# tictacmenthe/F2CNN

Measured on AMD Instinct MI355X. Metric: audio-seconds/sec through filterbank+envelope (HIP, 1 MI355X per rank); the +CNN figure of BASELINE's metric is value_with_cnn / blocks.cfg4, higher is better.
Workload: dtype f64 filter state + f64 utterance FFT + f32 row FFT; 1 GPU; cfg3: filterbank + Hilbert envelope + 50 Hz LPF in one call (f32 FFT), batch of 1000 x 1 s utterances per GPU, 128 channels, ENV1 (float64) out; channels=128, lpf_hz=50, launch_batch=1000, outputs_resident_in_hbm=True, parallelism=utterance-sharded x1, no collective, utterances_sent_back_by_the_accuracy_guard=0

## Files before the change

### f2cnn_amd/csrc/f2_fft13_merged.h

```cpp
#pragma once
template <int NT, int PTV>
__device__ __forceinline__ void fft13_pass12_merged(cpx<float>* lds, const cpx<float>* twl, int tid, cpx<float> (&v)[PTV]) {
    constexpr int LOG2H = 13;
    static_assert(NT == 512 && PTV >= 16 && plan_npass(LOG2H) == 4 && plan_bits(LOG2H, 1) == 3 && plan_bits(LOG2H, 2) == 2 &&
                      plan_bits(LOG2H, 0) == 4, "the 16-8-4-16 plan on 512 threads");
    constexpr int OFF2 = plan_tw_offset(LOG2H, 2) - plan_tw_offset(LOG2H, 1);
    const int l = tid & 63, hl = l >> 5;
    const int base8 = (l & 31) + 32 * (tid >> 6);
#pragma unroll
    for (int i = 0; i < 2; ++i) {
        const int b = base8 + 256 * (i + 2 * hl);
        const cpx<float>* src = lds + cpad(b);
#pragma unroll
        for (int j = 0; j < 8; ++j) v[i * 8 + j] = src[j * (1024 + 64)];
    }
    __syncthreads();
#pragma unroll
    for (int i = 0; i < 2; ++i) {
        dft<8>(&v[i * 8]);
        const cpx<float>* t1 = twl + (((base8 >> 4) + 16 * (i + 2 * hl)));
#pragma unroll
        for (int k = 1; k < 8; ++k) v[i * 8 + brev<8>(k)] = cmul(v[i * 8 + brev<8>(k)], t1[(k - 1) * 64]);
    }
#pragma unroll
    for (int i = 0; i < 2; ++i) {
        cpx<float>& A0 = v[i * 8 + brev<8>(0)];
        cpx<float>& B0 = v[i * 8 + brev<8>(4)];
        cpx<float>& A1 = v[i * 8 + brev<8>(1)];
        cpx<float>& B1 = v[i * 8 + brev<8>(5)];
        cpx<float>& A2 = v[i * 8 + brev<8>(2)];
        cpx<float>& B2 = v[i * 8 + brev<8>(6)];
        cpx<float>& A3 = v[i * 8 + brev<8>(3)];
        cpx<float>& B3 = v[i * 8 + brev<8>(7)];
        asm volatile("s_nop 1\n\t"
                     "v_permlane32_swap_b32 %0, %1\n\t"
                     "v_permlane32_swap_b32 %2, %3\n\t"
                     "v_permlane32_swap_b32 %4, %5\n\t"
                     "v_permlane32_swap_b32 %6, %7\n\t"
                     "v_permlane32_swap_b32 %8, %9\n\t"
                     "v_permlane32_swap_b32 %10, %11\n\t"
                     "v_permlane32_swap_b32 %12, %13\n\t"
                     "v_permlane32_swap_b32 %14, %15\n\t"
                     "s_nop 1"
                     : "+v"(A0.re), "+v"(B0.re), "+v"(A0.im), "+v"(B0.im), "+v"(A1.re), "+v"(B1.re), "+v"(A1.im), "+v"(B1.im),
                       "+v"(A2.re), "+v"(B2.re), "+v"(A2.im), "+v"(B2.im), "+v"(A3.re), "+v"(B3.re), "+v"(A3.im), "+v"(B3.im));
    }
    const int q = base8 & 15, plo = base8 >> 4;
    const cpx<float>* t2 = twl + OFF2 + plo;
#pragma unroll
    for (int k = 0; k < 4; ++k) {
        cpx<float> t[4] = {v[brev<8>(k)], v[8 + brev<8>(k)], v[brev<8>(k + 4)], v[8 + brev<8>(k + 4)]};
        dft<4>(t);
        const int pos = q + 16 * (k + 4 * hl) + 512 * plo;
        lds[cpad(pos)] = t[0];
#pragma unroll
        for (int k2 = 1; k2 < 4; ++k2) lds[cpad(pos + 128 * k2)] = cmul(t[brev<4>(k2)], t2[(k2 - 1) * 16]);
    }
    __syncthreads();
}

#define F2_SWAP8(OP, a0, b0, a1, b1, a2, b2, a3, b3, a4, b4, a5, b5, a6, b6, a7, b7)                                        \
    asm volatile("s_nop 1\n\t" OP " %0, %1\n\t" OP " %2, %3\n\t" OP " %4, %5\n\t" OP " %6, %7\n\t" OP " %8, %9\n\t" OP      \
                 " %10, %11\n\t" OP " %12, %13\n\t" OP " %14, %15\n\ts_nop 1"                                                \
                 : "+v"(a0), "+v"(b0), "+v"(a1), "+v"(b1), "+v"(a2), "+v"(b2), "+v"(a3), "+v"(b3), "+v"(a4), "+v"(b4),       \
                   "+v"(a5), "+v"(b5), "+v"(a6), "+v"(b6), "+v"(a7), "+v"(b7))
template <int NT, int PTV>
__device__ __forceinline__ void fft14_pass12_merged(cpx<float>* lds, const cpx<float>* twl, int tid, cpx<float> (&v)[PTV]) {
    constexpr int LOG2H = 14;
    static_assert(NT == 1024 && PTV >= 16 && plan_npass(LOG2H) == 4 && plan_bits(LOG2H, 0) == 4 && plan_bits(LOG2H, 1) == 4 &&
                      plan_bits(LOG2H, 2) == 2 && plan_bits(LOG2H, 3) == 4, "the 16-16-4-16 plan on 1024 threads");
    constexpr int OFF2 = plan_tw_offset(LOG2H, 2) - plan_tw_offset(LOG2H, 1);
    const int l = tid & 63, wv = tid >> 6;
    const int x = l & 15, jp = l >> 4;
    const int b = x + 16 * (wv + 16 * jp);
    const cpx<float>* src = lds + cpad(b);
#pragma unroll
    for (int j = 0; j < 16; ++j) v[j] = src[j * (1024 + 64)];
    __syncthreads();
    dft<16>(&v[0]);
    const cpx<float>* t1 = twl + (wv + 16 * jp);
#pragma unroll
    for (int k = 1; k < 16; ++k) v[brev<16>(k)] = cmul(v[brev<16>(k)], t1[(k - 1) * 64]);
#define F2_S(k) v[brev<16>(k)]
    F2_SWAP8("v_permlane32_swap_b32", F2_S(0).re, F2_S(8).re, F2_S(0).im, F2_S(8).im, F2_S(1).re, F2_S(9).re, F2_S(1).im, F2_S(9).im,
             F2_S(2).re, F2_S(10).re, F2_S(2).im, F2_S(10).im, F2_S(3).re, F2_S(11).re, F2_S(3).im, F2_S(11).im);
    F2_SWAP8("v_permlane32_swap_b32", F2_S(4).re, F2_S(12).re, F2_S(4).im, F2_S(12).im, F2_S(5).re, F2_S(13).re, F2_S(5).im,
             F2_S(13).im, F2_S(6).re, F2_S(14).re, F2_S(6).im, F2_S(14).im, F2_S(7).re, F2_S(15).re, F2_S(7).im, F2_S(15).im);
    F2_SWAP8("v_permlane16_swap_b32", F2_S(0).re, F2_S(4).re, F2_S(0).im, F2_S(4).im, F2_S(1).re, F2_S(5).re, F2_S(1).im, F2_S(5).im,
             F2_S(2).re, F2_S(6).re, F2_S(2).im, F2_S(6).im, F2_S(3).re, F2_S(7).re, F2_S(3).im, F2_S(7).im);
    F2_SWAP8("v_permlane16_swap_b32", F2_S(8).re, F2_S(12).re, F2_S(8).im, F2_S(12).im, F2_S(9).re, F2_S(13).re, F2_S(9).im,
             F2_S(13).im, F2_S(10).re, F2_S(14).re, F2_S(10).im, F2_S(14).im, F2_S(11).re, F2_S(15).re, F2_S(11).im, F2_S(15).im);
    const int kk0 = 4 * (jp & 1) + 8 * (jp >> 1);
    const cpx<float>* t2 = twl + OFF2 + wv;
#pragma unroll
    for (int k = 0; k < 4; ++k) {
        cpx<float> t[4] = {F2_S(k), F2_S(k + 4), F2_S(k + 8), F2_S(k + 12)};
        dft<4>(t);
        const int pos = x + 16 * (k + kk0) + 1024 * wv;
        lds[cpad(pos)] = t[0];
#pragma unroll
        for (int k2 = 1; k2 < 4; ++k2) lds[cpad(pos + 256 * k2)] = cmul(t[brev<4>(k2)], t2[(k2 - 1) * 16]);
    }
#undef F2_S
    __syncthreads();
}

template <int LOG2H, int NT, int PTV>
__device__ __forceinline__ void fft_pass0_pair(const cpx<float>* __restrict__ tw, int tid, cpx<float> (&va)[PTV], cpx<float> (&vb)[PTV]) {
    constexpr int R = 16, NB = (1 << LOG2H) / R;
    static_assert(NT == NB && PTV == R && plan_bits(LOG2H, 0) == 4, "one radix-16 butterfly per thread");
    dft<R>(&va[0]);
    dft<R>(&vb[0]);
    const cpx<float>* twq = tw + plan_tw_offset(LOG2H, 0) + tid;
    cpx<float> w[R];
    w[1] = twq[0];
    w[4] = twq[3 * NB];
    w[2] = cmul(w[1], w[1]);
    w[3] = cmul(w[2], w[1]);
    w[8] = cmul(w[4], w[4]);
    w[5] = cmul(w[4], w[1]);
    w[6] = cmul(w[4], w[2]);
    w[7] = cmul(w[4], w[3]);
    w[12] = cmul(w[8], w[4]);
    w[9] = cmul(w[8], w[1]);
    w[10] = cmul(w[8], w[2]);
    w[11] = cmul(w[8], w[3]);
    w[13] = cmul(w[12], w[1]);
    w[14] = cmul(w[12], w[2]);
    w[15] = cmul(w[12], w[3]);
#pragma unroll
    for (int k = 1; k < R; ++k) {
        va[brev<R>(k)] = cmul(va[brev<R>(k)], w[k]);
        vb[brev<R>(k)] = cmul(vb[brev<R>(k)], w[k]);
    }
}

template <int LOG2H, int PTV, int NT, bool T0REGS, int PASS = 1>
__device__ __forceinline__ void fft_remaining_passes(cpx<float>* lds, const cpx<float>* __restrict__ tw, const cpx<float>* twl, int tid,
                                                     cpx<float> (&v)[PTV]) {
    constexpr int NP = plan_npass(LOG2H);
    if constexpr (PASS < NP) {
        fft_pass<float, LOG2H, PASS, false, PASS == NP - 1, PTV, NT, false, T0REGS>(lds, tw, twl, tid, v);
        fft_remaining_passes<LOG2H, PTV, NT, T0REGS, PASS + 1>(lds, tw, twl, tid, v);
    }
}
template <int LOG2H, int PTV, int NT, bool T0REGS>
__device__ __forceinline__ void fft_from_pass0(cpx<float>* lds, const cpx<float>* __restrict__ tw, const cpx<float>* twl, int tid,
                                               cpx<float> (&v)[PTV]) {
#pragma unroll
    for (int k = 0; k < 16; ++k) lds[cpad(tid * 16 + k)] = v[brev<16>(k)];
    __syncthreads();
    if constexpr (LOG2H == 13) {
        fft13_pass12_merged<NT, PTV>(lds, twl, tid, v);
        fft_pass<float, 13, 3, false, true, PTV, NT, false, T0REGS>(lds, tw, twl, tid, v);
    } else if constexpr (LOG2H == 14) {
        fft14_pass12_merged<NT, PTV>(lds, twl, tid, v);
        fft_pass<float, 14, 3, false, true, PTV, NT, false, T0REGS>(lds, tw, twl, tid, v);
    } else {
        fft_remaining_passes<LOG2H, PTV, NT, T0REGS>(lds, tw, twl, tid, v);
    }
}

template <int PTV, int NT, bool T0REGS>
__device__ __forceinline__ void fft13_regs_to_regs(cpx<float>* lds, const cpx<float>* __restrict__ tw, const cpx<float>* twl, int tid,
                                                   cpx<float> (&v)[PTV]) {
    fft_pass<float, 13, 0, true, false, PTV, NT, false, T0REGS>(lds, tw, twl, tid, v);
    fft13_pass12_merged<NT, PTV>(lds, twl, tid, v);
    fft_pass<float, 13, 3, false, true, PTV, NT, false, T0REGS>(lds, tw, twl, tid, v);
}
```

### f2cnn_amd/csrc/f2_fft_lds.h

```cpp
#pragma once
#include <cmath>
#include <vector>

#include "f2_envelope_core.h"

namespace f2fft {

constexpr int THREADS13 = 512;
constexpr int MINWAVES13 = 4;
template <typename F>
constexpr int threads_for(int log2h) {
    return (log2h == 14 && sizeof(F) == 4) ? 1024 : (log2h == 13 && sizeof(F) == 4) ? THREADS13 : log2h >= 13 ? 512 : 256;
}
template <typename F, int LOG2H>
constexpr int threads_for() { return threads_for<F>(LOG2H); }
template <typename F, int LOG2H>
constexpr int min_waves_for() {
    return (sizeof(F) == 4 && LOG2H == 13) ? MINWAVES13 : (sizeof(F) == 4 && LOG2H == 14) ? 4 : 2;
}

template <typename F, int LOG2H>
constexpr bool derive_tw0() { return sizeof(F) == 4 && LOG2H >= 11 && LOG2H <= 14; }

constexpr int FUSE_HILBERT_MAX = 12;
template <typename F, int LOG2H>
constexpr bool fuse_hilbert() { return LOG2H >= 1 && LOG2H <= FUSE_HILBERT_MAX && sizeof(F) == 4; }

constexpr int plan_npass(int h, int p13 = 4) {
    return h == 0 ? 0 : h <= 5 ? 1 : h <= 10 ? ((h & 1) ? 3 : 2) : (h == 13 && p13 == 4) ? 4 : h == 14 ? 4 : 3;
}
constexpr int plan_bits(int h, int pass, int p13 = 4) {
    if (h <= 5) return h;
    if (h <= 10) return (h & 1) ? (pass == 1 ? 1 : (h - 1) / 2) : h / 2;
    if (h == 13 && p13 == 4) return pass == 1 ? 3 : pass == 2 ? 2 : 4;
    if (h == 14) return pass == 2 ? 2 : 4;
    const int a = h <= 13 ? 4 : 5;
    return pass == 1 ? h - 2 * a : a;
}
constexpr int plan_points_per_thread(int h, int nt, int p13 = 4) {
    int m = 1;
    for (int p = 0; p < plan_npass(h, p13); ++p) {
        const int R = 1 << plan_bits(h, p, p13);
        const int nb = (1 << h) / R;
        const int pts = ((nb + nt - 1) / nt) * R;
        m = pts > m ? pts : m;
    }
    return m;
}
constexpr int plan_shift(int h, int pass, int p13 = 4) {
    int s = 0;
    for (int i = 0; i < pass; ++i) s += plan_bits(h, i, p13);
    return s;
}
constexpr int plan_tw_count(int h, int pass, int p13 = 4) {
    const int R = 1 << plan_bits(h, pass, p13), S = 1 << plan_shift(h, pass, p13), H = 1 << h;
    return S * R == H ? 0 : (R - 1) * (H / R / S);
}
constexpr int plan_tw_offset(int h, int pass, int p13 = 4) {
    int o = 0;
    for (int i = 0; i < pass; ++i) o += plan_tw_count(h, i, p13);
    return o;
}
constexpr int plan_tw_total(int h, int p13 = 4) { return plan_tw_offset(h, plan_npass(h, p13), p13); }
constexpr int plan_tw_lds_count(int h, int p13 = 4) { return plan_npass(h, p13) >= 2 ? plan_tw_total(h, p13) - plan_tw_offset(h, 1, p13) : 0; }

__device__ __forceinline__ int cpad(int i) { return i + (i >> 4); }
constexpr int cpad_size(int h) { return h + (h >> 4) + 1; }

template <typename F, int LOG2H, int PASS, bool SRC_REGS, bool DST_REGS, int PTV, int NT, bool HILBERT = false,
          bool T0REGS = false, int P13 = 4>
__device__ __forceinline__ void fft_pass(cpx<F>* lds, const cpx<F>* __restrict__ tw, const cpx<F>* twl, int tid,
                                         cpx<F> (&v)[PTV]) {
    constexpr int H = 1 << LOG2H;
    constexpr int R = 1 << plan_bits(LOG2H, PASS, P13);
    constexpr int LOG2S = plan_shift(LOG2H, PASS, P13);
    constexpr int S = 1 << LOG2S;
    constexpr int NB = H / R;
    constexpr int ITER = (NB + NT - 1) / NT;
    constexpr bool LAST = (S * R == H);
    static_assert(ITER * R <= PTV, "register array too small");
    constexpr bool FULL = NB % NT == 0;
    const cpx<F>* __restrict__ twp = tw + plan_tw_offset(LOG2H, PASS, P13);
    if constexpr (!SRC_REGS) {
#pragma unroll
        for (int i = 0; i < ITER; ++i) {
            const int bf = tid + i * NT;
            if (FULL || bf < NB) {
                if constexpr (NB % 16 == 0) {
                    const cpx<F>* src = lds + cpad(bf);
#pragma unroll
                    for (int j = 0; j < R; ++j) v[i * R + j] = src[j * (NB + NB / 16)];
                } else {
#pragma unroll
                    for (int j = 0; j < R; ++j) v[i * R + j] = lds[cpad(bf + j * NB)];
                }
                if constexpr (HILBERT) {
                    const cpx<F>* __restrict__ V = tw + plan_tw_total(LOG2H, P13);
                    const F sc = F(1.0 / H);
#pragma unroll
                    for (int j = 0; j < R; ++j) {
                        const int m = bf + j * NB;
                        const cpx<F> zp = (NB % 16 == 0) ? (lds + cpad(H - bf))[-j * (NB + NB / 16)] : lds[cpad(H - m)];
                        const bool upper = 2 * m > H;
                        const cpx<F> vk = V[upper ? H - m : m];
                        const F cs = (upper ? -vk.re : vk.re) * sc, sn = -vk.im * sc;
                        const cpx<F> z = v[i * R + j];
                        const F wre = cs * zp.re - sn * z.im, wim = sn * z.re - cs * zp.im;
                        v[i * R + j] = {m == 0 ? F(0) : wre, m == 0 ? F(0) : -wim};
                    }
                }
            }
        }
        __syncthreads();
    }
#pragma unroll
    for (int i = 0; i < ITER; ++i) {
        const int bf = tid + i * NT;
        if (FULL || bf < NB) {
            dft<R>(&v[i * R]);
            if constexpr (!LAST) {
                const cpx<F>* twq = (PASS >= 1 ? twl + (plan_tw_offset(LOG2H, PASS, P13) - plan_tw_offset(LOG2H, 1, P13)) : twp) +
                                    (bf >> LOG2S);
                if constexpr (PASS == 0 && T0REGS && R == 16) {
                    cpx<F> w[R];
                    w[1] = twq[0];
                    w[4] = twq[3 * (NB / S)];
                    w[2] = cmul(w[1], w[1]);
                    w[3] = cmul(w[2], w[1]);
                    w[8] = cmul(w[4], w[4]);
                    w[5] = cmul(w[4], w[1]);
                    w[6] = cmul(w[4], w[2]);
                    w[7] = cmul(w[4], w[3]);
                    w[12] = cmul(w[8], w[4]);
                    w[9] = cmul(w[8], w[1]);
                    w[10] = cmul(w[8], w[2]);
                    w[11] = cmul(w[8], w[3]);
                    w[13] = cmul(w[12], w[1]);
                    w[14] = cmul(w[12], w[2]);
                    w[15] = cmul(w[12], w[3]);
#pragma unroll
                    for (int k = 1; k < R; ++k) v[i * R + brev<R>(k)] = cmul(v[i * R + brev<R>(k)], w[k]);
                } else {
#pragma unroll
                    for (int k = 1; k < R; ++k)
                        v[i * R + brev<R>(k)] = cmul(v[i * R + brev<R>(k)], twq[(k - 1) * (NB / S)]);
                }
            }
            if constexpr (!DST_REGS) {
                const int q = bf & (S - 1);
                const int base = q + (bf - q) * R;
                if constexpr (S % 16 == 0) {
                    cpx<F>* dst = lds + cpad(base);
#pragma unroll
                    for (int k = 0; k < R; ++k) dst[k * (S + S / 16)] = v[i * R + brev<R>(k)];
                } else {
#pragma unroll
                    for (int k = 0; k < R; ++k) lds[cpad(base + S * k)] = v[i * R + brev<R>(k)];
                }
            }
        }
    }
    if constexpr (!DST_REGS) __syncthreads();
}

template <typename F, int LOG2H, bool INVERSE, int PTV, int NT, bool T0REGS = false, int PASS = 0, int P13 = 4>
__device__ __forceinline__ void fft_all(cpx<F>* lds, const cpx<F>* __restrict__ tw, const cpx<F>* twl, int tid,
                                        cpx<F> (&v)[PTV]) {
    constexpr int NP = plan_npass(LOG2H, P13);
    if constexpr (PASS < NP) {
        constexpr bool SRC = !INVERSE && PASS == 0;
        constexpr bool DST = INVERSE && PASS == NP - 1;
// ... 46 lines not shown
```

### f2cnn_amd/csrc/f2_spectral.hip

```cpp
#include <algorithm>
#include <cmath>
#include <complex>
#include <thread>

#include "f2_fft_lds.h"

using namespace f2fft;

namespace {

typedef float f2_f4 __attribute__((ext_vector_type(4)));
constexpr int SPEC_GB = 16;

constexpr int KS_CGROUP = 32;
constexpr int KS_CGROUP_LONG = 8;
constexpr int KS_STORE_AUX = 2;
typedef unsigned int f2_u4 __attribute__((ext_vector_type(4)));
typedef unsigned int f2_u2 __attribute__((ext_vector_type(2)));
__device__ __forceinline__ __amdgpu_buffer_rsrc_t row_buffer(double* y, int n) {
    return __builtin_amdgcn_make_buffer_rsrc(y, 0, n * 8, 0x00020000);
}
__device__ __forceinline__ __amdgpu_buffer_rsrc_t row_buffer_uniform(double* y, int n) {
    const unsigned long long a = (unsigned long long)y;
    const unsigned lo = __builtin_amdgcn_readfirstlane((unsigned)a), hi = __builtin_amdgcn_readfirstlane((unsigned)(a >> 32));
    return row_buffer((double*)(((unsigned long long)hi << 32) | lo), __builtin_amdgcn_readfirstlane(n));
}
__device__ __forceinline__ void store_row_pair_inside(__amdgpu_buffer_rsrc_t r, int i0, double a, double b) {
    const f2_d2 v = {a, b};
    __builtin_amdgcn_raw_buffer_store_b128(__builtin_bit_cast(f2_u4, v), r, i0 * 8, 0, KS_STORE_AUX);
}
__device__ __forceinline__ void store_row_pair_buf(__amdgpu_buffer_rsrc_t r, int n, int i0, double a, double b) {
    if (i0 + 1 < n) {
        const f2_d2 v = {a, b};
        __builtin_amdgcn_raw_buffer_store_b128(__builtin_bit_cast(f2_u4, v), r, i0 * 8, 0, KS_STORE_AUX);
    } else if (i0 < n) {
        __builtin_amdgcn_raw_buffer_store_b64(__builtin_bit_cast(f2_u2, a), r, i0 * 8, 0, KS_STORE_AUX);
    }
}
__device__ __forceinline__ void store_row_pair_front(__amdgpu_buffer_rsrc_t r, int t0, double a, double b) {
    if (t0 >= 0) {
        const f2_d2 v = {a, b};
        __builtin_amdgcn_raw_buffer_store_b128(__builtin_bit_cast(f2_u4, v), r, t0 * 8, 0, KS_STORE_AUX);
    } else if (t0 == -1) {
        __builtin_amdgcn_raw_buffer_store_b64(__builtin_bit_cast(f2_u2, b), r, 0, 0, KS_STORE_AUX);
    }
}

struct LowpassConsts {
    float qf, b0f;
    float g1, g2, g4, g8;
    double gw, gblk;
};

template <int NT, int NBLK>
constexpr size_t lowpass_tab_lds_bytes() {
    return sizeof(float) * (2 * (size_t)NBLK * (NT / 64) + NBLK);
}

#define F2_DPP_STEP(CTRL)                                                                                                    \
    asm volatile("s_nop 1\n\t"                                                                                               \
                 "v_fmac_f32_dpp %0, %0, %16 " CTRL "\n\t"                                                                   \
                 "v_fmac_f32_dpp %1, %1, %16 " CTRL "\n\t"                                                                   \
                 "v_fmac_f32_dpp %2, %2, %16 " CTRL "\n\t"                                                                   \
                 "v_fmac_f32_dpp %3, %3, %16 " CTRL "\n\t"                                                                   \
                 "v_fmac_f32_dpp %4, %4, %16 " CTRL "\n\t"                                                                   \
                 "v_fmac_f32_dpp %5, %5, %16 " CTRL "\n\t"                                                                   \
                 "v_fmac_f32_dpp %6, %6, %16 " CTRL "\n\t"                                                                   \
                 "v_fmac_f32_dpp %7, %7, %16 " CTRL "\n\t"                                                                   \
                 "v_fmac_f32_dpp %8, %8, %16 " CTRL "\n\t"                                                                   \
                 "v_fmac_f32_dpp %9, %9, %16 " CTRL "\n\t"                                                                   \
                 "v_fmac_f32_dpp %10, %10, %16 " CTRL "\n\t"                                                                 \
                 "v_fmac_f32_dpp %11, %11, %16 " CTRL "\n\t"                                                                 \
                 "v_fmac_f32_dpp %12, %12, %16 " CTRL "\n\t"                                                                 \
                 "v_fmac_f32_dpp %13, %13, %16 " CTRL "\n\t"                                                                 \
                 "v_fmac_f32_dpp %14, %14, %16 " CTRL "\n\t"                                                                 \
                 "v_fmac_f32_dpp %15, %15, %16 " CTRL                                                                        \
                 : "+v"(sc[0]), "+v"(sc[1]), "+v"(sc[2]), "+v"(sc[3]), "+v"(sc[4]), "+v"(sc[5]), "+v"(sc[6]), "+v"(sc[7]),   \
                   "+v"(sc[8]), "+v"(sc[9]), "+v"(sc[10]), "+v"(sc[11]), "+v"(sc[12]), "+v"(sc[13]), "+v"(sc[14]), "+v"(sc[15]) \
                 : "v"(mult))

template <int NT, int NBLK, bool CHAINED = false, bool INSIDE_BUT_FIRST = false>
__device__ __forceinline__ float lowpass_pairs_store_tab(const float (&er)[NBLK], const float (&ei)[NBLK], const LowpassConsts& K,
                                                        const f2_f4* __restrict__ lptab, unsigned char* smem,
                                                        double* __restrict__ y, int n, int tid, int ibase = 0,
                                                        double* ychain = nullptr, int np = 0) {
    static_assert(NBLK == 16, "sixteen blocks: one DPP row chains them");
// ... 176 lines not shown
    asm volatile("s_nop 1\n\t"                                         \
                 "v_max_f32_dpp %0, %0, %0 " CTRL "\n\t"               \
                 "v_max_f32_dpp %1, %1, %1 " CTRL                       \
                 : "+v"(a), "+v"(b))
__device__ __forceinline__ void wave_max63x2(float& a, float& b) {
    F2_DPP_MAX2("row_shr:1 row_mask:0xf bank_mask:0xf bound_ctrl:0");
    F2_DPP_MAX2("row_shr:2 row_mask:0xf bank_mask:0xf bound_ctrl:0");
    F2_DPP_MAX2("row_shr:4 row_mask:0xf bank_mask:0xf bound_ctrl:0");
    F2_DPP_MAX2("row_shr:8 row_mask:0xf bank_mask:0xf bound_ctrl:0");
    F2_DPP_MAX2("row_bcast:15 row_mask:0xa bank_mask:0xf");
    F2_DPP_MAX2("row_bcast:31 row_mask:0xc bank_mask:0xf");
}
__device__ __forceinline__ float wave_max63(float v) {
    asm volatile("s_nop 1\n\t"
                 "v_max_f32_dpp %0, %0, %0 row_shr:1 row_mask:0xf bank_mask:0xf bound_ctrl:0\n\ts_nop 1\n\t"
                 "v_max_f32_dpp %0, %0, %0 row_shr:2 row_mask:0xf bank_mask:0xf bound_ctrl:0\n\ts_nop 1\n\t"
                 "v_max_f32_dpp %0, %0, %0 row_shr:4 row_mask:0xf bank_mask:0xf bound_ctrl:0\n\ts_nop 1\n\t"
                 "v_max_f32_dpp %0, %0, %0 row_shr:8 row_mask:0xf bank_mask:0xf bound_ctrl:0\n\ts_nop 1\n\t"
                 "v_max_f32_dpp %0, %0, %0 row_bcast:15 row_mask:0xa bank_mask:0xf\n\ts_nop 1\n\t"
                 "v_max_f32_dpp %0, %0, %0 row_bcast:31 row_mask:0xc bank_mask:0xf"
                 : "+v"(v));
    return v;
}

template <int R0, int NT, bool PADFIRST>
__device__ __forceinline__ float pad_residual(const cpx<float> (&v)[R0], int np, int tid, int odd, float gout) {
    if constexpr (PADFIRST) {
        return fmaxf(gout, 2 * tid + odd < np ? fabsf(v[brev<R0>(0)].re) : 0.f);
    } else {
        int jlim = (np - 2 * tid - odd + 2 * NT - 1) >> (__builtin_ctz(2 * NT));
        asm volatile("" : "+v"(jlim));
#pragma unroll
        for (int j = 0; j < R0 / 2; ++j) gout = fmaxf(gout, j < jlim ? fabsf(v[brev<R0>(j)].re) : 0.f);
        return gout;
    }
}

template <int NT, int NBLK, bool FIRSTONLY>
__device__ __forceinline__ void zero_front_padding(float (&er)[NBLK], float (&ei)[NBLK], int np, int tid) {
    int d = 2 * tid - np;
    asm volatile("" : "+v"(d));
#pragma unroll
    for (int jj = 0; jj < (FIRSTONLY ? 1 : NBLK / 2); ++jj) {
        er[jj] = d >= -2 * NT * jj ? er[jj] : 0.f;
        ei[jj] = d >= -2 * NT * jj - 1 ? ei[jj] : 0.f;
    }
}

#ifdef F2_STAMPS
#define F2_STAMP_STORE_ROW(st, N, out, row)                                                             \
    do {                                                                                                \
        if (threadIdx.x == 0 && (out))                                                                  \
            for (int k_ = 0; k_ < (N); ++k_) (out)[(size_t)(row) * (N) + k_] = (st)[k_];                \
    } while (0)
#else
#define F2_STAMP_STORE_ROW(st, N, out, row) \
    do {                                    \
    } while (0)
#endif

__device__ __forceinline__ void guard_decide(const SpecParams& P, const unsigned* guard, int b, int c) {
    const float gi = __uint_as_float(guard[0]), go = __uint_as_float(guard[1]), gl = __uint_as_float(guard[2]);
    const float den = P.lpf ? gl : gi;
    const bool flag = go > P.tol * den;
    if (flag) P.uflag[b] = 1;
    if (P.gdump) {
        float* g = P.gdump + ((size_t)b * (size_t)P.C + (size_t)c) * 4;
        g[0] = gi;
        g[1] = go;
        g[2] = gl;
        g[3] = flag ? 1.f : 0.f;
    }
}

template <int LOG2H, bool PADFIRST>
__global__ __launch_bounds__((threads_for<float, LOG2H>()), (min_waves_for<float, LOG2H>())) void k_spectral_envelope(
    const cpx<float>* __restrict__ Xall , const f2_f4* __restrict__ HUall,
    const cpx<float>* __restrict__ E , const float* __restrict__ rho_all ,
    const int64_t* __restrict__ offsets, const int* __restrict__ ulist, const cpx<float>* __restrict__ tw,
    const f2_f4* __restrict__ lptab, SpecParams P) {
    constexpr int NT = threads_for<float, LOG2H>();
    constexpr int H = 1 << LOG2H;
    constexpr int M = 2 * H;
    constexpr int CS = cpad_size(H);
    constexpr int R0 = 1 << plan_bits(LOG2H, 0);
    constexpr int NB0 = H / R0;
    static_assert(NB0 % NT == 0, "every thread owns whole butterflies of the first pass");
    constexpr int ITER0 = NB0 / NT;
    constexpr int PT = plan_points_per_thread(LOG2H, NT);
    constexpr int NBLK = ITER0 * R0;
    static_assert(PT == NBLK, "register shape");
    constexpr size_t LP = lowpass_tab_lds_bytes<NT, NBLK>();
    constexpr int LDS_BYTES = (int)((size_t)CS * 8 > LP ? (size_t)CS * 8 : LP);
    __shared__ __attribute__((aligned(16))) unsigned char smem[LDS_BYTES];
    constexpr int TWL = plan_tw_lds_count(LOG2H);
    __shared__ __attribute__((aligned(16))) cpx<float> twl[TWL > 0 ? TWL : 1];
    __shared__ unsigned guard[4];
    cpx<float>* lds = reinterpret_cast<cpx<float>*>(smem);

    const int tid = threadIdx.x;
    int u, c;
    row_decode<KS_CGROUP>(P, u, c);
    const int row_id = u * P.C + c;
    const float* __restrict__ rho_g = rho_all + (size_t)row_id * 8;
    const cpx<float>* __restrict__ Xu = Xall + (size_t)((unsigned long long)(unsigned)u * P.xpitch);
    const f2_f4* __restrict__ HUc = HUall + (size_t)((unsigned long long)(unsigned)c * P.tpitch);

    F2_STAMP_ARRAY(st, 8);
    F2_STAMP(st, 0);
    if (tid < 4) guard[tid] = 0u;

    static_assert(ITER0 == 1 && R0 == 16, "one radix-16 butterfly per thread in the first pass");
    constexpr int GB = SPEC_GB, NG = R0 / GB;
    cpx<float> yk[PT], v[PT];
    static_assert(NB0 == NT && plan_npass(LOG2H) >= 3, "fft_pass0_pair + fft_from_pass0");
    cpx<float> vo[PT];
    cpx<float> w0 = E[tid];
    constexpr int TWIT = (TWL + NT - 1) / NT;
    cpx<float> twr[TWIT > 0 ? TWIT : 1];
    {
        unsigned tw1 = plan_tw_offset(LOG2H, 1) * (unsigned)sizeof(cpx<float>);
        asm volatile("" : "+s"(tw1));
#pragma unroll
        for (int it = 0; it < TWIT; ++it) {
            const unsigned i = (it + 1) * NT <= TWL ? (unsigned)(tid + it * NT) : min((unsigned)(tid + it * NT), (unsigned)(TWL - 1));
            twr[it] = *reinterpret_cast<const cpx<float>*>(reinterpret_cast<const char*>(tw) + (i * (unsigned)sizeof(cpx<float>) + tw1));
        }
    }
    const cpx<float> XH = Xu[H];
    const f2_f4 HUH = HUc[H];
    float rho[8];
#pragma unroll
    for (int q = 0; q < 8; ++q) rho[q] = rho_g[q];
    cpx<float> Xl[2][GB];
    f2_f4 Hl[2][GB];
    unsigned kb8 = (unsigned)tid * (unsigned)sizeof(cpx<float>);
    asm volatile("" : "+v"(kb8));
    const __amdgpu_buffer_rsrc_t Xb = table_buffer(Xu, (H + 1) * (int)sizeof(cpx<float>)), HUb = table_buffer(HUc, (H + 1) * (int)sizeof(f2_f4));
    int b = 0;
#pragma unroll
    for (int qq = 0; qq < GB; ++qq) {
        const int q = qq == 0 ? 0 : qq == 1 ? GB - 1 : qq - 1;
        Xl[0][q] = lane_load<cpx<float>>(Xb, kb8, q * NB0);
        Hl[0][q] = lane_load<f2_f4>(HUb, 2 * kb8, q * NB0);
        __builtin_amdgcn_sched_barrier(0);
        if (qq == 0) {
            int u_late = u;
            asm volatile("" : "+s"(u_late));
            b = ulist[u_late];
        }
    }
    float nyq[6] = {XH.re, XH.im, HUH.x, HUH.y, HUH.z, HUH.w};
    asm volatile("" : "+s"(nyq[0]), "+s"(nyq[1]), "+s"(nyq[2]), "+s"(nyq[3]), "+s"(nyq[4]), "+s"(nyq[5]));
    asm volatile("" : "+s"(rho[0]), "+s"(rho[1]), "+s"(rho[2]), "+s"(rho[3]), "+s"(rho[4]), "+s"(rho[5]), "+s"(rho[6]), "+s"(rho[7]));
#pragma unroll
    for (int it = 0; it < TWIT; ++it) twl[(it + 1) * NT <= TWL ? tid + it * NT : min(tid + it * NT, TWL - 1)] = twr[it];
    asm volatile("" : "+s"(b));
    const int64_t off = offsets[b];
    const int n = (int)(offsets[b + 1] - off);
    const int np = M - n;
    double* __restrict__ y = P.env + ((size_t)P.C * (size_t)off + (size_t)c * (size_t)n);
#pragma unroll
    for (int g = 0; g < NG; ++g) {
        if (g + 1 < NG) {
#pragma unroll
            for (int q = 0; q < GB; ++q) {
                Xl[(g + 1) & 1][q] = lane_load<cpx<float>>(Xb, kb8, ((g + 1) * GB + q) * NB0);
                Hl[(g + 1) & 1][q] = lane_load<f2_f4>(HUb, 2 * kb8, ((g + 1) * GB + q) * NB0);
            }
        }
#pragma unroll
        for (int q = 0; q < GB; ++q) {
            const int j = g * GB + q;
            const cpx<float> wj = bin_w<R0>(w0, j);
            yk[j] = spectral_bin(Xl[g & 1][q], Hl[g & 1][q], wj, rho);
            vo[j] = {yk[j].re * wj.re + yk[j].im * wj.im, yk[j].re * wj.im - yk[j].im * wj.re};
#ifdef F2_STAMPS
            if (j == 0 || j == 7) {
                asm volatile("s_nop 0" : "+v"(yk[j].re), "+v"(yk[j].im));
                st[j == 0 ? 1 : 2] = __builtin_amdgcn_s_memrealtime();
                asm volatile("s_nop 0" : "+v"(yk[j].re));
            }
#endif
        }
        asm volatile("" : "+v"(kb8), "+v"(w0.re), "+v"(w0.im), "+v"(yk[g * GB].re), "+v"(yk[g * GB + GB - 1].re));
    }
#ifdef F2_STAMPS
    asm volatile("s_nop 0" : "+v"(yk[15].re), "+v"(yk[15].im));
    st[3] = __builtin_amdgcn_s_memrealtime();
    asm volatile("s_nop 0" : "+v"(yk[15].re));
#endif
    if (tid == 0) {
        const cpx<float> yh = spectral_bin(cpx<float>{nyq[0], nyq[1]}, f2_f4{nyq[2], nyq[3], nyq[4], nyq[5]}, cpx<float>{-1.f, 0.f}, rho);
        yk[0] = {yk[0].re, yh.re};
    }
    float er[NBLK], ei[NBLK];
    float gin = 0.f, gout = 0.f;
    constexpr bool T0R = derive_tw0<float, LOG2H>();
    {
#pragma unroll
        for (int j = 0; j < R0; ++j) v[j] = {yk[j].re, -yk[j].im};
        if (tid == 0) {
            v[0] = {0.5f * (yk[0].re + yk[0].im), 0.f};
            vo[0] = {0.5f * (yk[0].re - yk[0].im), 0.f};
        }
        F2_STAMP(st, 4);
        int tid_e = tid;
        asm volatile("" : "+v"(tid_e), "+v"(v[0].re), "+v"(vo[PT - 1].im));
        fft_pass0_pair<LOG2H, NT, PT>(tw, tid_e, v, vo);
        fft_from_pass0<LOG2H, PT, NT, T0R>(lds, tw, twl, tid_e, v);
        gout = pad_residual<R0, NT, PADFIRST>(v, np, tid, 0, gout);
#pragma unroll
        for (int j = 0; j < R0; ++j) {
            const cpx<float> a = v[brev<R0>(j)];
            er[j] = fsqrt(a.re * a.re + a.im * a.im);
        }
        fft_from_pass0<LOG2H, PT, NT, T0R>(lds, tw, twl, tid_e, vo);
        F2_STAMP(st, 5);
        gout = pad_residual<R0, NT, PADFIRST>(vo, np, tid, 1, gout);
#pragma unroll
        for (int j = 0; j < R0; ++j) {
            const cpx<float> a = vo[brev<R0>(j)];
            ei[j] = fsqrt(a.re * a.re + a.im * a.im);
        }
    }
    zero_front_padding<NT, NBLK, PADFIRST>(er, ei, np, tid);
#pragma unroll
    for (int jj = 0; jj < NBLK; ++jj) gin = fmaxf(gin, fmaxf(er[jj], ei[jj]));
    float glp = 0.f;
    wave_max63x2(gin, gout);
    if ((tid & 63) == 63) {
        __hip_atomic_fetch_max(&guard[0], __float_as_uint(gin), __ATOMIC_RELAXED, __HIP_MEMORY_SCOPE_WORKGROUP);
        __hip_atomic_fetch_max(&guard[1], __float_as_uint(gout), __ATOMIC_RELAXED, __HIP_MEMORY_SCOPE_WORKGROUP);
    }
    F2_STAMP(st, 6);
    if (!P.lpf) {
        const __amdgpu_buffer_rsrc_t yb = row_buffer(y, n);
#pragma unroll
        for (int jj = 0; jj < NBLK; ++jj) {
            const int t0 = 2 * (tid + NT * jj) - np;
            if ((PADFIRST && jj > 0) || jj >= NBLK / 2 || 2 * NT * jj >= np) store_row_pair_inside(yb, t0, (double)er[jj], (double)ei[jj]);
            else if (2 * NT * (jj + 1) > np) store_row_pair_front(yb, t0, (double)er[jj], (double)ei[jj]);
        }
    } else {
        glp = wave_max63(lowpass_pairs_store_tab<NT, NBLK, false, PADFIRST>(er, ei, P.lp, lptab, smem, y, n, tid, 0, nullptr, np));
    }
    if ((tid & 63) == 63) {
        if (P.lpf) __hip_atomic_fetch_max(&guard[2], __float_as_uint(glp), __ATOMIC_RELAXED, __HIP_MEMORY_SCOPE_WORKGROUP);
        if (__hip_atomic_fetch_add(&guard[3], 1u, __ATOMIC_ACQ_REL, __HIP_MEMORY_SCOPE_WORKGROUP) == (unsigned)(NT / 64 - 1))
            guard_decide(P, guard, b, c);
    }
    F2_STAMP(st, 7);
    F2_STAMP_STORE_ROW(st, 8, P.stamps, row_id);
}

constexpr int KSL_PARK_AUX = 0;
__device__ __forceinline__ int park_plane(int n, int bank, int r) {
    constexpr int MB = 8192;
    if (bank == 0) return n + r * MB;
    const int nb = n - 4 * MB;
    const int before = r == 0 ? 0 : r == 1 ? (nb + 3) >> 2 : r == 2 ? ((nb + 3) >> 2) + ((nb + 2) >> 2) : nb - (nb >> 2);
    return n + 4 * MB + before;
}
__global__ __launch_bounds__(1024, 4) void k_spectral_envelope_long(
    const cpx<float>* __restrict__ Xall, const f2_f4* __restrict__ HUall, const cpx<float>* __restrict__ E,
    const float* __restrict__ rho_all, const int64_t* __restrict__ offsets, const int* __restrict__ ulist,
    const cpx<float>* __restrict__ tw, const f2_f4* __restrict__ lptab, SpecParams P) {
    constexpr int LOG2Q = 14, NT = 1024, Q = 1 << LOG2Q, H = 2 * Q, M = 2 * H;
    static_assert(threads_for<float, LOG2Q>() == NT, "the 16-16-4-16 plan on 1024 threads");
    constexpr int CS = cpad_size(Q);
    constexpr int R0 = 16, NB0 = Q / R0, PT = 16, NBLK = 16;
    static_assert(NB0 == NT && plan_points_per_thread(LOG2Q, NT) == PT, "one radix-16 butterfly per thread in the first pass");
    constexpr size_t LP = lowpass_tab_lds_bytes<NT, NBLK>();
    constexpr int LDS_BYTES = (int)((size_t)CS * 8 > LP ? (size_t)CS * 8 : LP);
    __shared__ __attribute__((aligned(16))) unsigned char smem[LDS_BYTES];
    constexpr int TWL = plan_tw_lds_count(LOG2Q);
    __shared__ __attribute__((aligned(16))) cpx<float> twl[TWL];
    __shared__ unsigned guard[4];
    __shared__ double ychain;
    cpx<float>* lds = reinterpret_cast<cpx<float>*>(smem);

    const int tid = threadIdx.x;
    int u, c;
    row_decode<KS_CGROUP_LONG>(P, u, c);
    const int row_id = u * P.C + c;
    const int b = ulist[u];
    const int64_t off = offsets[b];
    const int n = (int)(offsets[b + 1] - off);
    double* __restrict__ y = P.env + ((size_t)P.C * (size_t)off + (size_t)c * (size_t)n);
    const float* __restrict__ rho = rho_all + (size_t)row_id * 8;
    const cpx<float>* __restrict__ Xu = Xall + (size_t)((unsigned long long)(unsigned)u * P.xpitch);
    const f2_f4* __restrict__ HUc = HUall + (size_t)((unsigned long long)(unsigned)c * P.tpitch);

    constexpr int TWIT = (TWL + NT - 1) / NT;
    cpx<float> twr[TWIT];
#pragma unroll
    for (int it = 0; it < TWIT; ++it) twr[it] = tw[plan_tw_offset(LOG2Q, 1) + ((it + 1) * NT <= TWL ? tid + it * NT : min(tid + it * NT, TWL - 1))];
    if (tid < 4) guard[tid] = 0u;
    if (tid == 0) ychain = 0.0;

    const unsigned zstep = ((unsigned)NB0 * (unsigned)n) & (M - 1);
    cpx<float> w0 = E[tid];
    cpx<float> z0 = E[((unsigned)tid * (unsigned)n) & (M - 1)];
    const cpx<float> zq = E[((unsigned)Q * (unsigned)n) & (M - 1)];
#pragma unroll
    for (int it = 0; it < TWIT; ++it)
        if ((it + 1) * NT <= TWL || tid + it * NT < TWL) twl[tid + it * NT] = twr[it];
    float yh = 0.f;
    if (tid == 0) yh = spectral_bin(Xu[H], HUc[H], cpx<float>{-1.f, 0.f}, cpx<float>{(n & 1) ? -1.f : 1.f, 0.f}, rho).re;
    constexpr bool T0R = derive_tw0<float, LOG2Q>();
    float gin = 0.f, gout = 0.f;
    unsigned kb = (unsigned)tid;
    F2_STAMP_ARRAY(st, 8);
    F2_STAMP(st, 0);
#pragma unroll 1
    for (int p = 0; p < 2; ++p) {
        cpx<float> v[PT], vo[PT];
        constexpr int GB = 4;
#pragma unroll
        for (int g = 0; g < R0 / GB; ++g) {
            cpx<float> Xl[2][GB];
            f2_f4 Hl[2][GB];
#pragma unroll
            for (int q = 0; q < GB; ++q) {
                Xl[0][q] = (Xu + (g * GB + q) * NB0)[kb];
                Hl[0][q] = (HUc + (g * GB + q) * NB0)[kb];
                Xl[1][q] = (Xu + Q + (g * GB + q) * NB0)[kb];
                Hl[1][q] = (HUc + Q + (g * GB + q) * NB0)[kb];
            }
#pragma unroll
            for (int q = 0; q < GB; ++q) {
                const int j = g * GB + q;
                const cpx<float> w = cmul(w0, E[j * NB0]);
                const cpx<float> z = cmul(z0, E[(j * zstep) & (M - 1)]);
                const cpx<float> ya = spectral_bin(Xl[0][q], Hl[0][q], w, z, rho);
                const cpx<float> yb2 = spectral_bin(Xl[1][q], Hl[1][q], cpx<float>{w.im, -w.re}, cmul(z, zq), rho);
                cpx<float> cp = {ya.re, -ya.im};
                if (j == 0 && tid == 0) cp = {0.5f * (ya.re + (p ? -yh : yh)), 0.f};
                const cpx<float> cr = p ? cpx<float>{-yb2.im, -yb2.re} : cpx<float>{yb2.re, -yb2.im};
                const cpx<float> sm = cp + cr, df = cp - cr;
                const cpx<float> w2 = cmul(w, w);
                v[j] = p ? cmul(sm, w) : sm;
                vo[j] = cmul(df, p ? cmul(w2, w) : w2);
            }
            asm volatile("" : "+v"(kb), "+v"(w0.re), "+v"(w0.im), "+v"(z0.re), "+v"(z0.im), "+v"(v[g * GB].re), "+v"(vo[g * GB + GB - 1].im));
        }
        int tid_e = tid;
        asm volatile("" : "+v"(tid_e), "+v"(v[0].re), "+v"(vo[PT - 1].im));
        if (p == 0) F2_STAMP(st, 1);
        else F2_STAMP(st, 3);
        fft_pass0_pair<LOG2Q, NT, PT>(tw, tid_e, v, vo);
#pragma unroll
        for (int half = 0; half < 2; ++half) {
            if (half == 0) fft_from_pass0<LOG2Q, PT, NT, T0R>(lds, tw, twl, tid_e, v);
            else fft_from_pass0<LOG2Q, PT, NT, T0R>(lds, tw, twl, tid_e, vo);
            const int r = p + 2 * half;
            const __amdgpu_buffer_rsrc_t yb = row_buffer_uniform(y, n);
            const int pv0 = 4 * (park_plane(n, 0, r) + tid), pv1 = 4 * (park_plane(n, 1, r) + tid);
#pragma unroll
            for (int j = 0; j < R0; ++j) {
                const cpx<float> a = half ? vo[brev<R0>(j)] : v[brev<R0>(j)];
                const float e = fsqrt(a.re * a.re + a.im * a.im);
                const bool in = 4 * (tid + NT * j) + r < n;
                __builtin_amdgcn_raw_buffer_store_b32(__float_as_uint(e), yb, in ? (j < 8 ? pv0 : pv1) : 0x7ffffff0, 4 * NT * (j & 7),
                                                      KSL_PARK_AUX);
                gin = fmaxf(gin, in ? e : 0.f);
                if (j >= 8 && 4 * NT * (j + 1) > n) gout = fmaxf(gout, in ? 0.f : fabsf(a.re));
            }
        }
        if (p == 0) F2_STAMP(st, 2);
        else F2_STAMP(st, 4);
    }
    gin = wave_max63(gin);
    gout = wave_max63(gout);
    if ((tid & 63) == 63) {
        atomicMax(&guard[0], __float_as_uint(gin));
        atomicMax(&guard[1], __float_as_uint(gout));
    }
    __builtin_amdgcn_fence(__ATOMIC_RELEASE, "workgroup");
    __syncthreads();
    __builtin_amdgcn_fence(__ATOMIC_ACQUIRE, "workgroup");
    float glp = 0.f;
#pragma unroll 1
    for (int sw = 0; sw < 2; ++sw) {
        const int ibase = sw * 2 * NT * NBLK;
        const __amdgpu_buffer_rsrc_t yb = row_buffer_uniform(y, n);
        float er[NBLK], ei[NBLK];
        const int rl = 2 * (tid & 1);
        const int pva = 4 * (park_plane(n, sw, rl) + (tid >> 1)), pvb = 4 * (park_plane(n, sw, rl + 1) + (tid >> 1));
#pragma unroll
        for (int jj = 0; jj < NBLK; ++jj) {
            const int i0 = ibase + 2 * (tid + NT * jj);
            er[jj] = __uint_as_float(__builtin_amdgcn_raw_buffer_load_b32(yb, i0 < n ? pva : 0x7ffffff0, 2 * NT * jj, KSL_PARK_AUX));
            ei[jj] = __uint_as_float(__builtin_amdgcn_raw_buffer_load_b32(yb, i0 + 1 < n ? pvb : 0x7ffffff0, 2 * NT * jj, KSL_PARK_AUX));
        }
        if (!P.lpf) {
            __syncthreads();
#pragma unroll
            for (int jj = 0; jj < NBLK; ++jj) store_row_pair_buf(yb, n, ibase + 2 * (tid + NT * jj), (double)er[jj], (double)ei[jj]);
        } else {
            glp = fmaxf(glp, lowpass_pairs_store_tab<NT, NBLK, true>(er, ei, P.lp, lptab, smem, y, n, tid, ibase, &ychain));
        }
        __syncthreads();
        if (sw == 0) F2_STAMP(st, 5);
        else F2_STAMP(st, 6);
    }
    if (P.lpf) glp = wave_max63(glp);
    if ((tid & 63) == 63) {
        if (P.lpf) __hip_atomic_fetch_max(&guard[2], __float_as_uint(glp), __ATOMIC_RELAXED, __HIP_MEMORY_SCOPE_WORKGROUP);
        if (__hip_atomic_fetch_add(&guard[3], 1u, __ATOMIC_ACQ_REL, __HIP_MEMORY_SCOPE_WORKGROUP) == (unsigned)(NT / 64 - 1))
            guard_decide(P, guard, b, c);
    }
    F2_STAMP(st, 7);
    F2_STAMP_STORE_ROW(st, 8, P.stamps, row_id);
}

template <typename WaveT, int LOG2HS, int LOGD, bool FRONT>
__global__ __launch_bounds__((threads_for<double, LOG2HS>())) void k_utterance_spectrum(const WaveT* __restrict__ wave,
                                                                                      const int64_t* __restrict__ offsets,
                                                                                      const int* __restrict__ ulist,
                                                                                      cpx<float>* __restrict__ X, int64_t xpitch,
                                                                                      cpx<double>* __restrict__ Xpart,
                                                                                      const cpx<double>* __restrict__ tw) {
    constexpr int LOG2H = LOG2HS;
    constexpr int D = 1 << LOGD;
    constexpr int NT = threads_for<double, LOG2H>();
    constexpr int H = 1 << LOG2H;
    constexpr int CS = cpad_size(H);
    constexpr int R0 = 1 << plan_bits(LOG2H, 0);
    constexpr int NB0 = H / R0;
    constexpr int ITER0 = (NB0 + NT - 1) / NT;
    constexpr int PT = plan_points_per_thread(LOG2H, NT);
    constexpr bool FULL0 = NB0 % NT == 0;
    __shared__ __attribute__((aligned(16))) cpx<double> lds[CS];
    constexpr int TWL = plan_tw_lds_count(LOG2H);
    __shared__ __attribute__((aligned(16))) cpx<double> twl[TWL > 0 ? TWL : 1];
    const cpx<double>* __restrict__ V = tw + plan_tw_total(LOG2H);
    const int tid = threadIdx.x;
// ... 463 lines not shown
```

Measured before the change: 215,500 audio-seconds/s.

## Use 32-element LDS padding with thread dealing for the 8K row FFT

Adds a Pad32 padding policy (one pad slot every 32 complex elements) for the LOG2H==13 spectral FFT path. It also adds a thread-to-butterfly dealing permutation for pass 0 so the contiguous 16-element stores stay conflict-free under the new padding. LDS accesses go through volatile 64-bit reads and writes so each complex value moves in a single instruction, and the stage-2 twiddles are hoisted out of the inner loop. The aim is fewer LDS bank conflicts and fewer split LDS instructions. The risk is that the volatile accesses block compiler scheduling, and the permuted thread mapping changes E and Xu table access patterns.

```diff
diff --git a/f2cnn_amd/csrc/f2_fft13_merged.h b/f2cnn_amd/csrc/f2_fft13_merged.h
--- a/f2cnn_amd/csrc/f2_fft13_merged.h
+++ b/f2cnn_amd/csrc/f2_fft13_merged.h
@@ -1,5 +1,5 @@
 #pragma once
-template <int NT, int PTV>
+template <int NT, int PTV, typename PAD = Pad16>
 __device__ __forceinline__ void fft13_pass12_merged(cpx<float>* lds, const cpx<float>* twl, int tid, cpx<float> (&v)[PTV]) {
     constexpr int LOG2H = 13;
     static_assert(NT == 512 && PTV >= 16 && plan_npass(LOG2H) == 4 && plan_bits(LOG2H, 1) == 3 && plan_bits(LOG2H, 2) == 2 &&
@@ -10,9 +10,9 @@
 #pragma unroll
     for (int i = 0; i < 2; ++i) {
         const int b = base8 + 256 * (i + 2 * hl);
-        const cpx<float>* src = lds + cpad(b);
+        const cpx<float>* src = lds + PAD::pad(b);
 #pragma unroll
-        for (int j = 0; j < 8; ++j) v[i * 8 + j] = src[j * (1024 + 64)];
+        for (int j = 0; j < 8; ++j) v[i * 8 + j] = lds_read<PAD>(src + j * PAD::step(1024));
     }
     __syncthreads();
 #pragma unroll
@@ -20,7 +20,7 @@
         dft<8>(&v[i * 8]);
         const cpx<float>* t1 = twl + (((base8 >> 4) + 16 * (i + 2 * hl)));
 #pragma unroll
-        for (int k = 1; k < 8; ++k) v[i * 8 + brev<8>(k)] = cmul(v[i * 8 + brev<8>(k)], t1[(k - 1) * 64]);
+        for (int k = 1; k < 8; ++k) v[i * 8 + brev<8>(k)] = cmul(v[i * 8 + brev<8>(k)], lds_read<PAD>(t1 + (k - 1) * 64));
     }
 #pragma unroll
     for (int i = 0; i < 2; ++i) {
@@ -47,14 +47,17 @@
     }
     const int q = base8 & 15, plo = base8 >> 4;
     const cpx<float>* t2 = twl + OFF2 + plo;
+    cpx<float> w2[4];
+#pragma unroll
+    for (int k2 = 1; k2 < 4; ++k2) w2[k2] = lds_read<PAD>(t2 + (k2 - 1) * 16);
 #pragma unroll
     for (int k = 0; k < 4; ++k) {
         cpx<float> t[4] = {v[brev<8>(k)], v[8 + brev<8>(k)], v[brev<8>(k + 4)], v[8 + brev<8>(k + 4)]};
         dft<4>(t);
-        const int pos = q + 16 * (k + 4 * hl) + 512 * plo;
-        lds[cpad(pos)] = t[0];
+        cpx<float>* dst = lds + PAD::pad(q + 64 * hl + 512 * plo) + PAD::step(16 * k);
+        lds_write<PAD>(dst, t[0]);
 #pragma unroll
-        for (int k2 = 1; k2 < 4; ++k2) lds[cpad(pos + 128 * k2)] = cmul(t[brev<4>(k2)], t2[(k2 - 1) * 16]);
+        for (int k2 = 1; k2 < 4; ++k2) lds_write<PAD>(dst + PAD::step(128 * k2), cmul(t[brev<4>(k2)], w2[k2]));
     }
     __syncthreads();
 }
@@ -135,6 +138,12 @@
     }
 }
 
+template <typename PAD>
+__device__ __forceinline__ int pass0_deal(int tid) {
+    if constexpr (PAD::LOG2PER == 5) return (tid & ~31) | ((tid & 15) << 1) | ((tid >> 4) & 1);
+    else return tid;
+}
+
 template <int LOG2H, int PTV, int NT, bool T0REGS, int PASS = 1>
 __device__ __forceinline__ void fft_remaining_passes(cpx<float>* lds, const cpx<float>* __restrict__ tw, const cpx<float>* twl, int tid,
                                                      cpx<float> (&v)[PTV]) {
@@ -144,15 +153,22 @@
         fft_remaining_passes<LOG2H, PTV, NT, T0REGS, PASS + 1>(lds, tw, twl, tid, v);
     }
 }
-template <int LOG2H, int PTV, int NT, bool T0REGS>
-__device__ __forceinline__ void fft_from_pass0(cpx<float>* lds, const cpx<float>* __restrict__ tw, const cpx<float>* twl, int tid,
+template <int LOG2H, int PTV, int NT, bool T0REGS, typename PAD = Pad16>
+__device__ __forceinline__ void fft_from_pass0(cpx<float>* lds, const cpx<float>* __restrict__ tw, const cpx<float>* twl, int tid, int t0,
                                                cpx<float> (&v)[PTV]) {
+    static_assert(PAD::LOG2PER == 4 || LOG2H == 13, "Pad32: the 16-8-4-16 plan only");
+    if constexpr (PAD::LOG2PER == 4) {
 #pragma unroll
-    for (int k = 0; k < 16; ++k) lds[cpad(tid * 16 + k)] = v[brev<16>(k)];
+        for (int k = 0; k < 16; ++k) lds[cpad(t0 * 16 + k)] = v[brev<16>(k)];
+    } else {
+        cpx<float>* dst = lds + PAD::pad(t0 * 16);
+#pragma unroll
+        for (int k = 0; k < 16; ++k) dst[k] = v[brev<16>(k)];
+    }
     __syncthreads();
     if constexpr (LOG2H == 13) {
-        fft13_pass12_merged<NT, PTV>(lds, twl, tid, v);
-        fft_pass<float, 13, 3, false, true, PTV, NT, false, T0REGS>(lds, tw, twl, tid, v);
+        fft13_pass12_merged<NT, PTV, PAD>(lds, twl, tid, v);
+        fft_pass<float, 13, 3, false, true, PTV, NT, false, T0REGS, 4, PAD>(lds, tw, twl, tid, v);
     } else if constexpr (LOG2H == 14) {
         fft14_pass12_merged<NT, PTV>(lds, twl, tid, v);
         fft_pass<float, 14, 3, false, true, PTV, NT, false, T0REGS>(lds, tw, twl, tid, v);
diff --git a/f2cnn_amd/csrc/f2_fft_lds.h b/f2cnn_amd/csrc/f2_fft_lds.h
--- a/f2cnn_amd/csrc/f2_fft_lds.h
+++ b/f2cnn_amd/csrc/f2_fft_lds.h
@@ -67,8 +67,40 @@
 __device__ __forceinline__ int cpad(int i) { return i + (i >> 4); }
 constexpr int cpad_size(int h) { return h + (h >> 4) + 1; }
 
+struct Pad16 {
+    static constexpr int LOG2PER = 4;
+    static constexpr bool SINGLE_READS = false;
+    static __device__ __forceinline__ int pad(int i) { return cpad(i); }
+    static constexpr int step(int s) { return s + (s >> 4); }
+    static constexpr int size(int h) { return cpad_size(h); }
+};
+struct Pad32 {
+    static constexpr int LOG2PER = 5;
+    static constexpr bool SINGLE_READS = true;
+    static __device__ __forceinline__ int pad(int i) { return i + (i >> 5); }
+    static constexpr int step(int s) { return s + (s >> 5); }
+    static constexpr int size(int h) { return h + (h >> 5) + 1; }
+};
+template <typename PAD, typename F>
+__device__ __forceinline__ cpx<F> lds_read(const cpx<F>* p) {
+    if constexpr (PAD::SINGLE_READS && sizeof(cpx<F>) == 8) {
+        const unsigned long long r = *(const volatile __attribute__((address_space(3))) unsigned long long*)p;
+        return __builtin_bit_cast(cpx<F>, r);
+    } else {
+        return *p;
+    }
+}
+template <typename PAD, typename F>
+__device__ __forceinline__ void lds_write(cpx<F>* p, cpx<F> x) {
+    if constexpr (PAD::SINGLE_READS && sizeof(cpx<F>) == 8) {
+        *(volatile __attribute__((address_space(3))) unsigned long long*)p = __builtin_bit_cast(unsigned long long, x);
+    } else {
+        *p = x;
+    }
+}
+
 template <typename F, int LOG2H, int PASS, bool SRC_REGS, bool DST_REGS, int PTV, int NT, bool HILBERT = false,
-          bool T0REGS = false, int P13 = 4>
+          bool T0REGS = false, int P13 = 4, typename PAD = Pad16>
 __device__ __forceinline__ void fft_pass(cpx<F>* lds, const cpx<F>* __restrict__ tw, const cpx<F>* twl, int tid,
                                          cpx<F> (&v)[PTV]) {
     constexpr int H = 1 << LOG2H;
@@ -79,6 +111,7 @@
     constexpr int ITER = (NB + NT - 1) / NT;
     constexpr bool LAST = (S * R == H);
     static_assert(ITER * R <= PTV, "register array too small");
+    static_assert(PAD::LOG2PER == 4 || (!SRC_REGS && DST_REGS && !HILBERT && NB % (1 << PAD::LOG2PER) == 0), "padding policy");
     constexpr bool FULL = NB % NT == 0;
     const cpx<F>* __restrict__ twp = tw + plan_tw_offset(LOG2H, PASS, P13);
     if constexpr (!SRC_REGS) {
@@ -86,7 +119,11 @@
         for (int i = 0; i < ITER; ++i) {
             const int bf = tid + i * NT;
             if (FULL || bf < NB) {
-                if constexpr (NB % 16 == 0) {
+                if constexpr (PAD::LOG2PER != 4) {
+                    const cpx<F>* src = lds + PAD::pad(bf);
+#pragma unroll
+                    for (int j = 0; j < R; ++j) v[i * R + j] = lds_read<PAD>(src + j * PAD::step(NB));
+                } else if constexpr (NB % 16 == 0) {
                     const cpx<F>* src = lds + cpad(bf);
 #pragma unroll
                     for (int j = 0; j < R; ++j) v[i * R + j] = src[j * (NB + NB / 16)];
diff --git a/f2cnn_amd/csrc/f2_spectral.hip b/f2cnn_amd/csrc/f2_spectral.hip
--- a/f2cnn_amd/csrc/f2_spectral.hip
+++ b/f2cnn_amd/csrc/f2_spectral.hip
@@ -2,6 +2,7 @@
 #include <cmath>
 #include <complex>
 #include <thread>
+#include <type_traits>
 
 #include "f2_fft_lds.h"
 
@@ -344,7 +345,8 @@
     constexpr int NT = threads_for<float, LOG2H>();
     constexpr int H = 1 << LOG2H;
     constexpr int M = 2 * H;
-    constexpr int CS = cpad_size(H);
+    using PAD = std::conditional_t<LOG2H == 13, Pad32, Pad16>;
+    constexpr int CS = PAD::size(H);
     constexpr int R0 = 1 << plan_bits(LOG2H, 0);
     constexpr int NB0 = H / R0;
     static_assert(NB0 % NT == 0, "every thread owns whole butterflies of the first pass");
@@ -361,6 +363,7 @@
     cpx<float>* lds = reinterpret_cast<cpx<float>*>(smem);
 
     const int tid = threadIdx.x;
+    const int t0 = pass0_deal<PAD>(tid);
     int u, c;
     row_decode<KS_CGROUP>(P, u, c);
     const int row_id = u * P.C + c;
@@ -377,7 +380,7 @@
     cpx<float> yk[PT], v[PT];
     static_assert(NB0 == NT && plan_npass(LOG2H) >= 3, "fft_pass0_pair + fft_from_pass0");
     cpx<float> vo[PT];
-    cpx<float> w0 = E[tid];
+    cpx<float> w0 = E[t0];
     constexpr int TWIT = (TWL + NT - 1) / NT;
     cpx<float> twr[TWIT > 0 ? TWIT : 1];
     {
@@ -396,7 +399,7 @@
     for (int q = 0; q < 8; ++q) rho[q] = rho_g[q];
     cpx<float> Xl[2][GB];
     f2_f4 Hl[2][GB];
-    unsigned kb8 = (unsigned)tid * (unsigned)sizeof(cpx<float>);
+    unsigned kb8 = (unsigned)t0 * (unsigned)sizeof(cpx<float>);
     asm volatile("" : "+v"(kb8));
     const __amdgpu_buffer_rsrc_t Xb = table_buffer(Xu, (H + 1) * (int)sizeof(cpx<float>)), HUb = table_buffer(HUc, (H + 1) * (int)sizeof(f2_f4));
     int b = 0;
@@ -469,15 +472,16 @@
         F2_STAMP(st, 4);
         int tid_e = tid;
         asm volatile("" : "+v"(tid_e), "+v"(v[0].re), "+v"(vo[PT - 1].im));
-        fft_pass0_pair<LOG2H, NT, PT>(tw, tid_e, v, vo);
-        fft_from_pass0<LOG2H, PT, NT, T0R>(lds, tw, twl, tid_e, v);
+        const int t0_e = pass0_deal<PAD>(tid_e);
+        fft_pass0_pair<LOG2H, NT, PT>(tw, t0_e, v, vo);
+        fft_from_pass0<LOG2H, PT, NT, T0R, PAD>(lds, tw, twl, tid_e, t0_e, v);
         gout = pad_residual<R0, NT, PADFIRST>(v, np, tid, 0, gout);
 #pragma unroll
         for (int j = 0; j < R0; ++j) {
             const cpx<float> a = v[brev<R0>(j)];
             er[j] = fsqrt(a.re * a.re + a.im * a.im);
         }
-        fft_from_pass0<LOG2H, PT, NT, T0R>(lds, tw, twl, tid_e, vo);
+        fft_from_pass0<LOG2H, PT, NT, T0R, PAD>(lds, tw, twl, tid_e, t0_e, vo);
         F2_STAMP(st, 5);
         gout = pad_residual<R0, NT, PADFIRST>(vo, np, tid, 1, gout);
 #pragma unroll
@@ -614,8 +618,8 @@
         fft_pass0_pair<LOG2Q, NT, PT>(tw, tid_e, v, vo);
 #pragma unroll
         for (int half = 0; half < 2; ++half) {
-            if (half == 0) fft_from_pass0<LOG2Q, PT, NT, T0R>(lds, tw, twl, tid_e, v);
-            else fft_from_pass0<LOG2Q, PT, NT, T0R>(lds, tw, twl, tid_e, vo);
+            if (half == 0) fft_from_pass0<LOG2Q, PT, NT, T0R>(lds, tw, twl, tid_e, tid_e, v);
+            else fft_from_pass0<LOG2Q, PT, NT, T0R>(lds, tw, twl, tid_e, tid_e, vo);
             const int r = p + 2 * half;
             const __amdgpu_buffer_rsrc_t yb = row_buffer_uniform(y, n);
             const int pv0 = 4 * (park_plane(n, 0, r) + tid), pv1 = 4 * (park_plane(n, 1, r) + tid);
```

New measurement: 217,600 audio-seconds/s, median of 6. 1.01x the previous value.
